# kamerkaya/SUPerman

Measured on AMD Instinct MI355X. Metric: Gray-code subset-steps/sec (dense n=40, d=0.5) at 1/2/4/8 MI355X; rel-err vs CPU, higher is better.
Workload: dtype f64; 1 GPU; dense Ryser/Gray-code exact permanent (-p4/-p6 path), n=40 d=0.50 (double/40_0.50_0), 2^39 Gray steps per step; n=40, kernel_request=dense, preprocessing=0, jit=1, walk=segmented (pattern-specialised), parallelism=dp1: contiguous wave-chunk shards + one RCCL all-reduce

## Files before the change

superman_amd/csrc/codescan.cpp:

```cpp
#include <amd_comgr/amd_comgr.h>
#include <elf.h>

#include <algorithm>
#include <cstring>
#include <map>
#include <string>
#include <string_view>
#include <vector>

#include "engine.hpp"

namespace sup {

namespace {

struct Inst {
  uint64_t addr = 0, size = 0;
  std::string text;
  int64_t target = -1;
};

struct DisCtx {
  const char* bytes = nullptr;
  uint64_t base = 0, len = 0;
// ... 66 lines not shown

bool starts(const std::string& s, const char* p) { return s.compare(0, std::strlen(p), p) == 0; }

bool is_f64_valu(const std::string& t) {
  return starts(t, "v_add_f64") || starts(t, "v_mul_f64") || starts(t, "v_fma_f64") || starts(t, "v_fmac_f64");
}
bool is_scratch(const std::string& t) { return starts(t, "scratch_") || starts(t, "buffer_"); }
bool is_readlane(const std::string& t) { return starts(t, "v_readlane"); }

}

int scan_code_object(const std::vector<char>& co, const char* kernel, CodeScan* out) {
  CodeScan r;
  r.vgprs = (int)meta_value(co, ".vgpr_count");
  r.vgpr_spills = (int)meta_value(co, ".vgpr_spill_count");
  r.scratch_bytes = (int)meta_value(co, ".private_segment_fixed_size");
  if (r.vgprs < 0 || r.vgpr_spills < 0 || r.scratch_bytes < 0) {
    set_error("code object: no register / scratch counts in its metadata");
    return SUP_EHIP;
  }
  const char* bytes = nullptr;
  uint64_t fa = 0, fs = 0, sa = 0, sl = 0;
  if (!find_function(co, kernel, &bytes, &fa, &fs, &sa, &sl) || fs == 0) {
    set_error(std::string("code object: kernel symbol ") + kernel + " not found");
    return SUP_EHIP;
  }
  DisCtx ctx;
  ctx.bytes = bytes, ctx.base = sa, ctx.len = sl;
  amd_comgr_disassembly_info_t dis;
  if (amd_comgr_create_disassembly_info("amdgcn-amd-amdhsa--gfx950", read_cb, print_cb, annot_cb, &dis) !=
      AMD_COMGR_STATUS_SUCCESS) {
    set_error("amd_comgr_create_disassembly_info failed");
    return SUP_EHIP;
  }
  std::vector<Inst> ins;
  int rc = SUP_OK;
  for (uint64_t a = fa; a < fa + fs;) {
    ctx.text.clear();
    ctx.target = -1;
    uint64_t sz = 0;
    if (amd_comgr_disassemble_instruction(dis, a, &ctx, &sz) != AMD_COMGR_STATUS_SUCCESS || sz == 0) {
      set_error("code object: disassembly failed");
      rc = SUP_EHIP;
      break;
    }
    Inst in;
    in.addr = a, in.size = sz;
    size_t p = ctx.text.find_first_not_of(" \t");
    in.text = p == std::string::npos ? std::string() : ctx.text.substr(p);
    const bool branch = starts(in.text, "s_branch") || starts(in.text, "s_cbranch");
    in.target = branch ? ctx.target : -1;
    ins.push_back(std::move(in));
    a += sz;
  }
  amd_comgr_destroy_disassembly_info(dis);
  if (rc) return rc;
  for (const Inst& in : ins) r.scratch_insts += is_scratch(in.text);
  r.insts = (int)ins.size();

  std::map<uint64_t, int> at;
  for (size_t i = 0; i < ins.size(); ++i) at[ins[i].addr] = (int)i;
  std::vector<char> leader(ins.size() + 1, 0);
  leader[0] = 1;
  for (size_t i = 0; i < ins.size(); ++i) {
    const Inst& in = ins[i];
    const bool ends = in.target >= 0 || starts(in.text, "s_endpgm") || starts(in.text, "s_setpc");
    if (ends) leader[i + 1] = 1;
    if (in.target >= 0) {
      auto it = at.find((uint64_t)in.target);
      if (it == at.end()) {
        set_error("code object: branch target outside the kernel");
        return SUP_EHIP;
      }
      leader[it->second] = 1;
    }
  }
  std::vector<int> bstart, block_of(ins.size());
  for (size_t i = 0; i < ins.size(); ++i) {
    if (leader[i]) bstart.push_back((int)i);
    block_of[i] = (int)bstart.size() - 1;
  }
  const int B = (int)bstart.size();
  std::vector<std::vector<int>> succ(B), pred(B);
  std::vector<int> bf64(B, 0), bscr(B, 0), blen(B, 0), brl(B, 0);
  for (int b = 0; b < B; ++b) {
    const int lo = bstart[b], hi = b + 1 < B ? bstart[b + 1] : (int)ins.size();
    for (int i = lo; i < hi; ++i)
      bf64[b] += is_f64_valu(ins[i].text), bscr[b] += is_scratch(ins[i].text), brl[b] += is_readlane(ins[i].text);
    blen[b] = hi - lo;
    const Inst& last = ins[hi - 1];
    auto add = [&](int to) {
      if (to >= 0 && to < B) succ[b].push_back(to), pred[to].push_back(b);
    };
    if (last.target >= 0) add(block_of[at[(uint64_t)last.target]]);
    const bool uncond = starts(last.text, "s_branch") || starts(last.text, "s_endpgm") || starts(last.text, "s_setpc");
    if (!uncond && hi < (int)ins.size()) add(b + 1);
  }
  std::vector<int> order, rpo_num(B, -1);
  {
    std::vector<char> seen(B, 0);
    std::vector<std::pair<int, size_t>> st{{0, 0}};
    seen[0] = 1;
    while (!st.empty()) {
      auto& [v, k] = st.back();
      if (k < succ[v].size()) {
        const int w = succ[v][k++];
        if (!seen[w]) seen[w] = 1, st.push_back({w, 0});
      } else {
        order.push_back(v);
        st.pop_back();
      }
    }
    std::reverse(order.begin(), order.end());
    for (size_t i = 0; i < order.size(); ++i) rpo_num[order[i]] = (int)i;
  }
  std::vector<int> idom(B, -1);
  idom[0] = 0;
  auto intersect = [&](int a, int b) {
    while (a != b) {
      while (rpo_num[a] > rpo_num[b]) a = idom[a];
      while (rpo_num[b] > rpo_num[a]) b = idom[b];
    }
    return a;
  };
  for (bool changed = true; changed;) {
    changed = false;
    for (int v : order) {
      if (v == 0) continue;
      int nd = -1;
      for (int p : pred[v])
        if (rpo_num[p] >= 0 && idom[p] >= 0) nd = nd < 0 ? p : intersect(p, nd);
      if (nd >= 0 && idom[v] != nd) idom[v] = nd, changed = true;
    }
  }
  auto dominates = [&](int h, int v) {
    if (rpo_num[v] < 0) return false;
    for (;;) {
      if (v == h) return true;
      if (v == 0) return false;
      v = idom[v];
    }
  };
  std::map<int, std::vector<char>> loops;
  for (int u = 0; u < B; ++u)
    for (int h : succ[u]) {
      if (!dominates(h, u)) continue;
      std::vector<char>& body = loops[h];
      if (body.empty()) body.assign(B, 0);
      body[h] = 1;
      std::vector<int> work;
      if (!body[u]) body[u] = 1, work.push_back(u);
      while (!work.empty()) {
        const int v = work.back();
        work.pop_back();
        for (int p : pred[v])
          if (!body[p]) body[p] = 1, work.push_back(p);
      }
    }
  r.loops = (int)loops.size();
  std::map<int, int> f64;
  for (auto& [h, body] : loops) {
    int s = 0;
    for (int b = 0; b < B; ++b) s += body[b] ? bf64[b] : 0;
    f64[h] = s;
  }
  int walk = -1;
  for (auto& [h, body] : loops) {
    bool outer = false;
    for (auto& [h2, body2] : loops)
      if (h2 != h && body[h2] && 2 * f64[h2] >= f64[h]) outer = true;
    if (!outer && (walk < 0 || f64[h] > f64[walk])) walk = h;
  }
  if (walk >= 0) {
    const std::vector<char>& body = loops[walk];
    r.loop_f64 = f64[walk];
    r.loop_scratch = 0;
    r.loop_insts = 0;
    r.loop_readlane = 0;
    for (int b = 0; b < B; ++b)
      if (body[b]) r.loop_scratch += bscr[b], r.loop_insts += blen[b], r.loop_readlane += brl[b];
  }
  *out = r;
  return SUP_OK;
}

}
```

superman_amd/csrc/engine.hpp:

```cpp
#pragma once
#include <stdint.h>
#include <cstdio>
#include <memory>
#include <mutex>
#include <functional>
#include <string>
#include <vector>

#include "../../include/superman.h"
#include "kernels.hpp"

namespace sup {

void set_error(const std::string& msg);
const char* last_error();
bool env_on(const char* name, bool dflt);

int to_double(const void* mat, sup_dtype t, int n, std::vector<double>& out);

void nw_start(const double* A, int n, double* x0, double* p0);

constexpr int kMaxCachedBits = 4;

enum SegCensus {
  kCenXAdd = 0,
  kCenCopy,
  kCenOuter,
  kCenInner,
  kCenD,
  kCenAcc,
  kCenLane,
  kCenSharedAdd,
  kCenSharedCopy,
  kCenSharedForm,
  kCenHiAdd,
  kCenHiCopy,
  kCenHiForm,
  kCenStart,
  kSegCensusN
};

struct Layout {
  int L;
  int m;
  int h;
  bool fixed = false;
  int cc_cap = kMaxCachedBits;
  uint64_t chunks() const { return 1ull << h; }
};
Layout default_layout(int n);
Layout layout_with_walk(int n, int walk_log2);

struct ProdTree {
  std::vector<int> item_row;
  std::vector<uint32_t> item_sig;
  int tail_lo = 0, tail_hi = 0;
  std::vector<int> a, b;
  std::vector<uint32_t> sig;
  std::vector<uint8_t> item_live, node_live;
  int items() const { return (int)item_row.size(); }
  int K() const { return (int)a.size(); }
  int root() const { return K() ? items() + K() - 1 : (items() ? 0 : -1); }
  uint32_t root_sig() const { return K() ? sig.back() : (items() ? item_sig[0] : 0u); }
};

struct Plan {
  int n = 0;
  int NP = 0;
  WalkKind kind = kWalkDense;
  Layout lay{};
  std::vector<int> rowperm;
  std::vector<int> colmap;
  std::vector<double> cols;
  std::vector<double> x0;
  std::vector<int> nblk;
  std::vector<uint64_t> rowmask;
  uint64_t umask = 0;
  uint64_t chunk_ends = 0;
  std::vector<int> seg_start;
  std::vector<std::vector<int>> touched;
  std::vector<int> sub_start;
  int seg_b = 0;
  std::vector<int> dyn_rows;
  ProdTree outer_tree;
  ProdTree inner_tree;
  bool lds = false;
  bool integral = false;
  int seg_cc = 0;
  double seg_ops = 0.0;
  double seg_model_ops = 0.0;
  int seg_hi = 0;
  double seg_census[kSegCensusN] = {};
  double seg_skip = 0.0;
  int seg_regs = 0;
  int seg_budget = 0;
  std::vector<int> jofs;
  std::vector<double> jtab;
  size_t seg_cbase = 0;
  bool start_tab_on = false;
  std::vector<double> start_tab;
  int seg_kp = 4;
  std::string jit_src;
  uint64_t jit_key = 0;
  uint64_t uid = 0;
  std::vector<int> seg_order;
  bool seg_loop_scratch = false;
};

struct SegChoice {
  std::vector<int> order;
  int b = 0;
  int budget = 0;
  int cc_cap = kMaxCachedBits;
  int hi = 0;
};

int make_plan(const double* A, int n, WalkKind kind, bool identity_map, const Layout& lay, Plan& P,
              const SegChoice* choice = nullptr);

std::vector<int> greedy_walk_order(const double* A, int n, int count);
bool skip_walk_order(const double* A, int n, const Layout& lay, std::vector<int>& out,
                     const std::vector<int>* baseline, double factor);
int improve_sparse_plan(const double* A, int n, const Layout& lay, Plan& P);
int plan_threads();

std::vector<int> seg_walk_order(const double* A, int n, int m, int count, int* b_out, int cc_cap = kMaxCachedBits);
double seg_skip_estimate(const double* A, int n, const std::vector<int>& order, int m, int samples);
double seg_skip_fraction_plan(const Plan& P, int samples);
std::vector<int> seg_row_order(const double* A, int n, const std::vector<int>& walk);
int build_seg(Plan& P, int fixed_budget = 0, int fixed_hi = 0);
bool seg_choice_load(uint64_t key, int* m, SegChoice* c);
bool seg_choice_exists(uint64_t key);
double seg_cold_model(int n);
double seg_cold_predict(int n);
void seg_cost_store(int n, double seconds);
double seg_cost_ratio_load();
void seg_choice_store(uint64_t key, int m, const SegChoice& c);
int auto_decision_load(uint64_t key);
int auto_decision_store(uint64_t key, int seg);
uint64_t jit_toolchain_hash();
int seg_static_bits(int m);
double seg_cx(const Plan& P, int r, uint32_t S);
double seg_cy(const Plan& P, int r, uint32_t S);
double seg_walk_cost(const Plan& P);
int jit_occupancy(int dev, const Plan& P, int* blocks_per_cu, double* compile_ms);
int jit_launch(int dev, const Plan& P, const WalkParams& p, int grid, hipStream_t s);
int jit_compile_only(const Plan& P, double* compile_ms);
struct CodeScan {
  int vgprs = -1, vgpr_spills = -1, scratch_bytes = -1;
  int insts = 0, scratch_insts = 0, loops = 0;
  int loop_scratch = -1, loop_f64 = 0, loop_insts = 0;
  int loop_readlane = 0;
};
int scan_code_object(const std::vector<char>& code, const char* kernel, CodeScan* out);
int jit_code_scan(const Plan& P, CodeScan* out);
double jit_compile_ms_thread();

double walk_cost(const Plan& P);
double walk_seconds(const Plan& P, double steps);

int plan_for(const double* A, int n, sup_kernel kernel, const Layout& lay, Plan& P, int jit = -1, int ndev = 1,
             int dev = 0);
int plan_for_shared(const double* A, int n, sup_kernel kernel, const Layout& lay, std::shared_ptr<const Plan>& P,
                    int jit = -1, int ndev = 1, int dev = 0, bool keep = true);

struct RangeResult {
  double partial = 0.0;
  double kernel_ms = 0.0;
  uint64_t visited = 0;
  int grid = 0;
  double compile_ms = 0.0;
};

int run_item_queue(uint64_t nitems, int takers, const std::function<int(int, uint64_t)>& take);
int run_range(int dev, const Plan& P, uint64_t c0, uint64_t c1, bool want_visited, RangeResult& r,
              double* slot = nullptr);
struct LaunchGeom {
  unsigned group, tail_group;
  uint64_t tail_begin, grid;
  unsigned tail_ticket;
};
LaunchGeom walk_geometry(uint64_t count, uint64_t resident_blocks, uint64_t waves_per_block, bool seg,
                         int force_group = 0, int force_tail = -1, uint64_t group_cap = 64);
constexpr int kMaxBatchLeaves = 32;
constexpr int kMaxBatchLeafChunkBits = 26;
static_assert((uint64_t)kMaxBatchLeaves << kMaxBatchLeafChunkBits <= (1ull << 32),
              "leaf batches must fit 32-bit chunk indices");
bool batchable(const Plan& a, const Plan& b);
int run_range_batch(int dev, const std::vector<const Plan*>& plans, std::vector<double>& partial, double* kernel_ms);

double pairwise_host(const std::vector<double>& v);

int device_count(int* n);
constexpr int kCtxLanes = 8;
void set_ctx_lane(int lane);
int ctx_lane();
void set_defer_timing(bool on);
int kernel_time(int dev, double* total_ms, uint64_t* launches);
int phys_device(int dev);
hipError_t select_device(int dev);
int check_device(int dev, const char* what);
uint64_t device_checks_passed();
#ifndef SUP_HIP
#define SUP_HIP(call)                                                                  \
  do {                                                                                 \
    hipError_t e_ = (call);                                                            \
    if (e_ != hipSuccess) {                                                            \
      set_error(std::string(#call) + ": " + hipGetErrorString(e_));                    \
      return SUP_EHIP;                                                                 \
    }                                                                                  \
  } while (0)
#endif

#define SUP_ON_DEVICE(dev, what)                 \
  do {                                           \
    const int rc_ = check_device((dev), (what)); \
    if (rc_) return rc_;                         \
  } while (0)
int warm_devices(int first, int count, int n);
int rccl_physical_devices(const std::vector<int>& devs, std::vector<int>& phys);

struct SchedResult {
  double total = 0.0;
  double kernel_ms = 0.0;
  uint64_t visited = 0;
  int devices = 0;
  int grid = 0;
  int cpu_items = 0;
  double compile_ms = 0.0;
  int items_resumed = 0;
  std::vector<double> dev_partials;
};
int schedule(const Plan& P, sup_sched sched, const sup_opts& o, uint64_t c0, uint64_t c1,
             SchedResult& out);
struct Checkpoint {
// ... 223 lines not shown
```

superman_amd/csrc/jit.cpp:

```cpp
#include <dlfcn.h>
#include <hip/hiprtc.h>
#include <sched.h>
#include <spawn.h>
#include <sys/stat.h>
#include <sys/wait.h>
#include <unistd.h>

#include <cerrno>

#include <algorithm>
#include <cstring>
#include <fstream>
#include <iterator>
#include <atomic>
#include <chrono>
#include <cmath>
#include <cstdio>
#include <cstdlib>
#include <map>
#include <queue>
#include <memory>
#include <condition_variable>
#include <mutex>
#include <sstream>
// ... 228 lines not shown
    const double bd = best < 0 ? 0.0 : dlt[best];
    if (!took_hi && (best < 0 || (bd > 1e-9 && regs <= budget_hi))) out(*fit_hi, ops, regs), took_hi = true;
    if (best < 0 || (bd > 1e-9 && regs <= budget)) break;
    heap.pop();
    V[best].live = false;
    ++ver[best];
    ops += bd, regs -= V[best].store;
    for (int p = V[best].parent; p >= 0; p = V[p].parent) {
      V[p].F += (double)V[p].cop / V[best].cop * V[best].F;
      if (V[p].live) {
        push(p);
        break;
      }
    }
    stack.assign(1, best);
    while (!stack.empty()) {
      const int u = stack.back();
      stack.pop_back();
      for (int k : V[u].kids)
        if (k >= 0) {
          if (V[k].live) push(k);
          else stack.push_back(k);
        }
    }
  }
  if (!took_hi) out(*fit_hi, ops, regs);
  out(f, ops, regs);
  return f;
}

std::atomic<long> g_fit_calls{0};
int search_budget() {
  static const int b = std::getenv("SUP_JIT_SEARCH_BUDGET") ? std::atoi(std::getenv("SUP_JIT_SEARCH_BUDGET")) : kRegsMax;
  return b;
}

int max_cached() {
  const char* e = std::getenv("SUP_JIT_MAXCC");
  return e ? std::max(0, std::min(kMaxCachedBits, std::atoi(e))) : kMaxCachedBits;
}

SegFit seg_best(const SegRows& R, int cc_max, int regs_max = kRegsMax) {
  ++g_fit_calls;
  SegFit best;
  double bscore = 1e300;
  for (int cc = 0; cc <= std::min(cc_max, std::max(0, R.b - 1)); ++cc) {
    SegFit hi;
    SegFit lo = seg_fit(R, cc, kRegs3, regs_max, &hi);
    for (SegFit* f : {&lo, &hi}) {
      if (f->regs > regs_max && cc > 0) continue;
      const double score = f->ops * (f->regs <= kRegs3 ? 1.0 : kOcc2Penalty) * (f->regs > regs_max ? 2.0 : 1.0);
      if (score < bscore) bscore = score, best = std::move(*f);
    }
  }
  return best;
}

SegRows seg_rows_of(const double* A, int n, const std::vector<int>& walk, int b) {
  SegRows R;
  R.n = n, R.m = (int)walk.size();
  const std::vector<int> order = seg_row_order(A, n, walk);
  auto nz = [&](int row, int c) { return A[(size_t)row * n + c] != 0.0; };
  R.touched.assign(R.m, {});
  std::vector<char> any1(n, 0);
  for (int k = 0; k < R.m; ++k)
    for (int j = 0; j < n; ++j)
      if (nz(order[j], walk[k])) {
        R.touched[k].push_back(j);
        if (k >= 1) any1[j] = 1;
      }
  R.len0 = (int)R.touched[0].size();
  R.s_end = 0;
  while (R.s_end < R.len0 && any1[R.s_end]) ++R.s_end;
  R.r_end = R.len0;
  while (R.r_end < n && any1[R.r_end]) ++R.r_end;
  seg_rows_finish(R, b);
  return R;
}

double seg_score(const SegFit& f) { return f.ops * (f.regs <= kRegs3 ? 1.0 : kOcc2Penalty); }

constexpr double kMaxBlockBytes = 40.0 * 1024.0;
double seg_block_bytes(const SegFit& f, int b) { return 1.25 * 8.0 * 2.0 * f.ops * (double)(1u << b); }

std::vector<int> seg_b_candidates(int m) {
  std::vector<int> v;
  if (const char* e = std::getenv("SUP_JIT_B")) {
    v.push_back(std::min(m - 1, std::max(3, std::min(8, std::atoi(e)))));
    return v;
  }
  for (int b = 5; b <= 8; ++b) {
    const int bb = std::min(m - 1, b);
    if (v.empty() || v.back() != bb) v.push_back(bb);
  }
  return v;
}

}

int seg_static_bits(int m) {
  int b = 5;
  if (const char* e = std::getenv("SUP_JIT_B")) b = std::max(3, std::min(8, std::atoi(e)));
  return std::min(m - 1, b);
}

double seg_walk_cost(const Plan& P) { return P.seg_ops; }

int plan_threads() {
  int t = (int)std::max(1u, std::thread::hardware_concurrency());
  if (const char* e = std::getenv("OMP_NUM_THREADS")) t = std::min(t, std::max(1, std::atoi(e)));
  return std::min(t, 16);
}

void parallel_tasks(size_t count, const std::function<void(size_t)>& fn, int max_threads = 1 << 20) {
  std::atomic<size_t> next{0};
  auto worker = [&]() {
    for (size_t i = next++; i < count; i = next++) fn(i);
  };
  std::vector<std::thread> th;
  for (int t = 1; t < std::min({plan_threads(), (int)count, max_threads}); ++t) th.emplace_back(worker);
  worker();
  for (auto& t : th) t.join();
}

int seg_search_starts(int n) {
  if (const char* e = std::getenv("SUP_JIT_STARTS")) return std::max(1, std::atoi(e));
  return std::ldexp(1.0, n - 1) * (2.0 * n + 1.0) / 3.7e13 >= 1.0 ? 32 : 3;
}

std::vector<int> seg_walk_order(const double* A, int n, int m, int count, int* b_out, int cc_cap) {
  cc_cap = std::min(cc_cap, max_cached());
  const int nb = n - 1;
  m = std::min(m, nb);
  count = std::min(std::max(count, m), nb);
  std::vector<int> nnz(n, 0);
  for (int c = 0; c < nb; ++c)
    for (int i = 0; i < n; ++i) nnz[c] += A[(size_t)i * n + c] != 0.0;
  auto extend = [&](std::vector<int> order, int upto) {
    std::vector<char> used(n, 0), placed(n, 0);
    for (int c : order) {
      used[c] = 1;
      for (int i = 0; i < n; ++i) placed[i] |= A[(size_t)i * n + c] != 0.0;
    }
    while ((int)order.size() < upto) {
      int best = -1, bnew = 1 << 30;
      for (int c = 0; c < nb; ++c) {
        if (used[c]) continue;
        int nw = 0;
        for (int i = 0; i < n; ++i) nw += !placed[i] && A[(size_t)i * n + c] != 0.0;
        if (nw < bnew || (nw == bnew && nnz[c] < nnz[best])) best = c, bnew = nw;
      }
      used[best] = 1;
      order.push_back(best);
      for (int i = 0; i < n; ++i) placed[i] |= A[(size_t)i * n + best] != 0.0;
    }
    return order;
  };
  auto cost = [&](const std::vector<int>& o, int b) {
    if (nnz[o[0]] == 0) return 1e300;
    if (m < 3) return 0.0;
    const SegFit f = seg_best(seg_rows_of(A, n, std::vector<int>(o.begin(), o.begin() + m), b), cc_cap,
                              search_budget());
    return seg_block_bytes(f, b) > kMaxBlockBytes ? 1e300 : seg_score(f);
  };
  if (m == 0) {
    if (b_out) *b_out = 0;
// ... 936 lines not shown
    auto tree_init = [&](int ti, int v) {
      const ProdTree& t = tr(ti);
      if (t.tail_hi > t.tail_lo)
        o << "      const double " << (ti == 0 ? "Ro" : (v ? "Cy" : "Cx")) << " = "
          << tree(t.tail_lo, t.tail_hi, v ? "y" : "x") << ";\n";
      for (int i = 0; i < t.K(); ++i)
        if (this->nlive(ti, v, i))
          for (uint32_t S : submasks(t.sig[i] & ccm))
            o << "      double " << nname(ti, v, i, S) << " = " << iopnd(ti, v, t.a[i], S) << " * "
              << iopnd(ti, v, t.b[i], S) << ";\n";
    };
    tree_init(0, 0);
    o << "      double acc = 0.0;\n";
    o << "      uint32_t vis = 0;\n";
    if (P.outer_tree.tail_hi > P.outer_tree.tail_lo)
      o << "      if (__builtin_amdgcn_ballot_w64(SUP_LANE() < " << (1u << L) << "u && Ro != 0.0) != 0) {\n";
    else
      o << "      {\n";
    o << "      vis = " << (1u << m) << "u;\n";
    tree_init(1, 0);
    tree_init(1, 1);
    if (P.inner_tree.root() >= 0)
      for (uint32_t S : submasks(inner_root_csig()))
        o << "      double " << dname(S) << " = " << dexpr([&](int v, int id) { return iopnd(1, v, id, S); })
          << ";\n";
    else
      o << "      double D0 = 0.0;\n";
    {
      const std::string U = top(0, 0, 0);
      o << "      acc = " << (U.empty() ? dname(0) : dname(0) + " * " + U) << ";\n";
    }
    o << "      double tot = 0.0;\n";
    if (trace) o << "      asm volatile(\"\" : \"+v\"(acc));\n      tr_sc += __builtin_amdgcn_s_memtime() - tr_s;\n      ++tr_n;\n";
    const int u = std::max(0, std::min(P.seg_hi, m - 1 - b));
    const unsigned U = 1u << u;
    const size_t start_end = o.str().size();
    if (u > 0) {
      hi_loop(Q, U, u);
    } else {
    o << "      for (uint32_t q = 0; q < " << Q << "u; ++q) {\n";
    const char* ind = "        ";
    o << ind << "const char* jt = (const char*)opaque_c(p.jtab, 0u);\n";
    o << ind << "const uint32_t ng = q & 1u;\n";
    {
      std::vector<Item> items;
      for (unsigned st = 1; st < B; ++st) {
        const int pb = __builtin_ctz(st), k = pb + 1;
        if (pb >= cc && !P.touched[k].empty())
          step_items(items, "jt", pb < b - 1 ? off_const(k, (st >> (pb + 1)) & 1u) : off_dyn(k, "ng"),
                     P.touched[k], false, step_class(k, b));
        items.push_back({accumulate_text(st & 1u, state(st)), {}});
        body[kCenAcc] += 1.0;
      }
      emit_items(items, ind);
    }
    body[kCenAcc] += 1.0;
    if (Q > 1) {
      o << ind << "if (q + 1u < " << Q << "u) {\n";
      o << ind << "  const uint32_t kk = (uint32_t)__builtin_ctz(q + 1u);\n";
      o << ind << "  const uint32_t ngd = ((q + 1u) >> (kk + 1u)) & 1u;\n";
      {
        std::vector<Item> items;
        step_items(items, "(const char*)opaque_c(p.cols, 0u)",
                   "(2u * (" + std::to_string(L + b + 1) + "u + kk) + ngd) * " + std::to_string(P.NP * 8) + "u",
                   P.dyn_rows, true, P.seg_b, kSharedStep);
        items.push_back({accumulate_text(false, 0u), {}});
        emit_items(items, "          ");
      }
      o << ind << "  tot += acc;\n" << ind << "  acc = 0.0;\n";
      body[kCenLane] += 1.0;
      o << ind << "}\n";
    }
    o << "      }\n";
    }
    {
      const double steps = 2.0 * (double)U * (double)B;
      double walk = 0.0;
      for (int c = 0; c < kCenStart; ++c) census[c] = body[c] / steps, walk += body[c];
      const std::string init = o.str().substr(start_begin, start_end - start_begin);
      const double start_ops = count_sub(init, " + ") + count_sub(init, " * ") + count_sub(init, " - ") +
                               count_sub(init, "__builtin_fma(") + 7.0 +
                               (double)n * ((double)L + (P.start_tab_on ? 0.0 : 0.5 * (double)(n - 1 - L - m)));
      census[kCenStart] = std::ldexp(start_ops, -m);
      block_bytes = 1.25 * 8.0 * walk;
    }
    o << "      acc = tot + acc;\n";
    o << "      if (((uint32_t)ga ^ (uint32_t)__builtin_popcount(SUP_LANE())) & 1u) acc = -acc;\n";
    o << "      }\n";
    o << "      const uint32_t lane = SUP_LANE();\n";
    o << "      const double part = wave_sum(lane < " << (1u << L) << "u ? acc : 0.0);\n";
    o << "      if (lane == j) s_keep[wv][j] = part, s_vkeep[wv][j] = vis;\n";
    o << "    }\n";
    o << "    __builtin_amdgcn_fence(__ATOMIC_RELEASE, \"wavefront\");\n";
    o << "    __builtin_amdgcn_wave_barrier();\n";
    o << "    __builtin_amdgcn_fence(__ATOMIC_ACQUIRE, \"wavefront\");\n";
    o << "    const uint32_t lane = SUP_LANE();\n";
    o << "    chunk_store(base, len, s_keep[wv][lane], s_vkeep[wv][lane]);\n";
    o << "    __builtin_amdgcn_wave_barrier();\n";
    o << "  }\n";
    if (trace)
      o << "  if (p.trace && SUP_LANE() == 0) {\n"
        << "    unsigned long long* t = p.trace + 8ull * (blockIdx.x * " << kBlock / 64 << "u + wv);\n"
        << "    t[0] = tr_r0; t[1] = __builtin_amdgcn_s_memrealtime(); t[2] = tr_c0;\n"
        << "    t[3] = __builtin_amdgcn_s_memtime(); t[4] = tr_n; t[5] = tr_sc;\n"
        << "  }\n";
    o << "}\n";
    o << "}  // namespace sup\n";
    return o.str();
  }
};

const char* const kJitOpts[] = {"--offload-arch=gfx950", "-O3", "-std=c++17", "-ffp-contract=off"};
constexpr int kJitNopts = 4;

}

std::vector<std::string> jit_opts() {
  std::vector<std::string> v(kJitOpts, kJitOpts + kJitNopts);
  if (const char* e = std::getenv("SUP_JIT_SCHED"))
    if (*e) v.push_back("-mllvm"), v.push_back(std::string("-amdgpu-sched-strategy=") + e);
  if (const char* e = std::getenv("SUP_JIT_OPAQUE_R2"))
    if (std::atoi(e)) v.push_back("-DSUP_OPAQUE_BEFORE_OFFSET=1");
  return v;
}

namespace {

uint64_t fnv1a(const std::string& s, uint64_t h = 1469598103934665603ull) {
  for (unsigned char c : s) h = (h ^ c) * 1099511628211ull;
  return h;
}

std::string hiprtc_version() {
  static const std::string v = [] {
    int major = 0, minor = 0;
    if (hiprtcVersion(&major, &minor) != HIPRTC_SUCCESS) return std::string("hiprtc ?");
    std::string r = "hiprtc " + std::to_string(major) + "." + std::to_string(minor) + " hip " + std::to_string(HIP_VERSION);
    Dl_info di;
    if (dladdr(reinterpret_cast<void*>(&hiprtcCreateProgram), &di) && di.dli_fname) {
      const char* slash = std::strrchr(di.dli_fname, '/');
      r += std::string(" ") + (slash ? slash + 1 : di.dli_fname);
      std::ifstream f(di.dli_fname, std::ios::binary);
      if (f) {
        std::string bytes((std::istreambuf_iterator<char>(f)), std::istreambuf_iterator<char>());
        char hx[40];
        std::snprintf(hx, sizeof hx, " %zu %016llx", bytes.size(), (unsigned long long)fnv1a(bytes));
        r += hx;
      }
    }
    return r;
  }();
  return v;
}

}

uint64_t toolchain_hash_impl() {
  std::string key;
  for (const std::string& opt : jit_opts()) key += "\n//" + opt;
  key += std::string("\n//") + kWalkCommonSrc + kWalkParamsSrc;
  key += "\n//" + hiprtc_version();
  return fnv1a(key);
}

namespace {

uint64_t jit_source_key(const std::string& src) {
// ... 24 lines not shown
        for (int j = 0; j < n; ++j) x[j] += col[j];
      }
    }
  });
}

int build_seg(Plan& P, int fixed_budget, int fixed_hi) {
  const int n = P.n, L = P.lay.L, m = P.lay.m;
  if (m < 3) {
    set_error("segmented walk needs >= 3 walk bits");
    return SUP_EINVAL;
  }
  if (P.cols.empty()) return SUP_EINVAL;
  P.start_tab.clear();
  P.start_tab_on = !std::getenv("SUP_JIT_NO_START_TAB") && P.lay.m <= kStartTabMaxWalkBits &&
                   (double)P.lay.chunks() * P.NP * sizeof(double) <= (double)kStartTabMaxBytes;
  P.touched.assign(m, {});
  P.seg_start.assign(1, 0);
  std::vector<char> seen(n, 0);
  int R = 0;
  for (int k = 0; k < m; ++k) {
    const double* col = P.cols.data() + (size_t)(2 * (L + k)) * P.NP;
    for (int j = 0; j < n; ++j)
      if (col[j] != 0.0) {
        P.touched[k].push_back(j);
        if (!seen[j]) seen[j] = 1, ++R;
      }
    if (R > P.seg_start.back()) P.seg_start.push_back(R);
  }
  for (int j = 0; j < R; ++j)
    if (!seen[j]) {
      set_error("segmented walk: rows are not in first-touch order");
      return SUP_EINVAL;
    }
  if (P.touched[0].empty()) {
    set_error("segmented walk: walk column 0 has no nonzero");
    return SUP_EINVAL;
  }
  {
    const int len0 = P.seg_start[1];
    std::vector<char> got(len0, 0);
    int cnt = 0;
    P.sub_start.assign(1, 0);
    for (int k = 1; k < m; ++k) {
      for (int r : P.touched[k])
        if (r < len0 && !got[r]) {
          if (r != cnt) {
            set_error("segmented walk: segment 0 rows are not in sub-segment order");
            return SUP_EINVAL;
          }
          got[r] = 1, ++cnt;
        }
      if (cnt > P.sub_start.back()) P.sub_start.push_back(cnt);
    }
  }
  if (P.seg_b < 1 || P.seg_b > m - 1) {
    P.seg_b = seg_static_bits(m);
    if (!std::getenv("SUP_JIT_B")) {
      double best = 1e300;
      for (const int cb : seg_b_candidates(m)) {
        SegRows R;
        R.n = n, R.m = m, R.touched = P.touched;
        R.len0 = P.seg_start[1], R.s_end = P.sub_start.back(), R.r_end = P.seg_start.back();
        seg_rows_finish(R, cb);
        const SegFit f = seg_best(R, std::min(max_cached(), P.lay.cc_cap));
        const double sc = seg_block_bytes(f, cb) > kMaxBlockBytes ? 1e300 : seg_score(f);
        if (sc < best - 1e-12) best = sc, P.seg_b = cb;
      }
    }
  }
  P.dyn_rows.clear();
  {
    std::vector<char> in(n, 0);
    for (int k = P.seg_b + 1; k < m; ++k)
      for (int r : P.touched[k]) in[r] = 1;
    for (int j = 0; j < n; ++j)
      if (in[j]) P.dyn_rows.push_back(j);
  }
  SegRows SR;
  SR.n = n, SR.m = m, SR.touched = P.touched;
  SR.len0 = P.seg_start[1], SR.s_end = P.sub_start.back(), SR.r_end = P.seg_start.back();
  seg_rows_finish(SR, P.seg_b);
  const int cc_cap = std::min(max_cached(), P.lay.cc_cap);
  auto finish = [&SR, &cc_cap, n, L, m](Plan& Q, int budget, int hi) {
    SegFit f;
    if (const char* e = std::getenv("SUP_JIT_CC"))
      f = seg_fit(SR, std::max(0, std::min({std::atoi(e), SR.b - 1, kMaxCachedBits})), budget);
    else f = seg_best(SR, cc_cap, budget);
    if (const char* e = std::getenv("SUP_JIT_STORAGE")) f = seg_fit(SR, f.cc, std::max(0, std::atoi(e)));
    Q.outer_tree = std::move(f.outer);
    Q.inner_tree = std::move(f.inner);
    Q.seg_cc = f.cc;
    Q.seg_model_ops = f.ops;
    Q.seg_regs = f.regs;
    Q.seg_budget = budget;
    Q.jofs.assign(m, 0);
    Q.jtab.clear();
    for (int k = 0; k < m; ++k) {
      const std::vector<int>& t = Q.touched[k];
      const size_t blk = (t.size() + 7) & ~(size_t)7;
      Q.jofs[k] = (int)Q.jtab.size();
      Q.jtab.resize(Q.jtab.size() + 2 * std::max<size_t>(blk, 8), 0.0);
      for (size_t i = 0; i < t.size(); ++i) {
        Q.jtab[Q.jofs[k] + i] = Q.cols[(size_t)(2 * (L + k)) * Q.NP + t[i]];
        Q.jtab[Q.jofs[k] + blk + i] = Q.cols[(size_t)(2 * (L + k) + 1) * Q.NP + t[i]];
      }
    }
    Q.seg_cbase = Q.jtab.size();
    Q.seg_kp = 4;
    if (const char* e = std::getenv("SUP_JIT_KP")) Q.seg_kp = std::max(1, std::atoi(e));
    const int hi_max = std::min(3, m - 1 - Q.seg_b);
    if (const char* e = std::getenv("SUP_JIT_HI")) hi = std::max(0, std::min(3, std::atoi(e)));
    bool neg_zero = false;
    for (int j = 0; j < n; ++j) neg_zero = neg_zero || (Q.x0[j] == 0.0 && std::signbit(Q.x0[j]));
    if (neg_zero) hi = 0;
    auto generate = [&Q](int h, std::string* src) {
      Q.seg_hi = h;
      auto g = std::make_unique<Gen>(Q);
      *src = g->source();
      return g;
    };
    auto total = [](const Gen& g) {
      double ops = 0.0;
      for (int c = 0; c < kCenStart; ++c) ops += g.census[c];
      return ops;
    };
    int taken = hi < 0 ? 0 : std::min(hi, hi_max);
    std::string src;
    std::unique_ptr<Gen> g = generate(taken, &src);
    for (int h = hi < 0 ? hi_max : 0; h > 0; --h) {
      std::string s2;
      std::unique_ptr<Gen> gh = generate(h, &s2);
      if (gh->block_bytes <= kMaxBlockBytes && total(*gh) < total(*g)) {
        g = std::move(gh), src = std::move(s2), taken = h;
        break;
      }
    }
    Q.seg_hi = taken;
    Q.jit_src = std::move(src);
    for (int c = 0; c < kSegCensusN; ++c) Q.seg_census[c] = g->census[c];
    Q.seg_ops = total(*g);
    {
      const std::vector<double> t = g->tail();
      Q.jtab.insert(Q.jtab.end(), t.begin(), t.end());
    }
    Q.jit_key = jit_source_key(Q.jit_src);
  };
  const char* env_budget = std::getenv("SUP_JIT_BUDGET");
  const int hi_unchecked = fixed_budget > 0 ? fixed_hi : 0;
  if (env_budget) fixed_budget = std::max(1, std::atoi(env_budget));
  finish(P, fixed_budget > 0 ? fixed_budget : kRegsMax, hi_unchecked);
  const bool fixed = fixed_budget > 0 || std::getenv("SUP_JIT_REGMAX") || std::getenv("SUP_JIT_STORAGE") ||
                     std::getenv("SUP_JIT_CC") || std::getenv("SUP_JIT_NOVERIFY");
  const double walk_s = std::ldexp(1.0, n - 1) * P.seg_ops / 3.7e13;
  if (fixed && std::getenv("SUP_JIT_VERBOSE")) {
    CodeScan s;
    const int rc = jit_code_scan(P, &s);
    std::fprintf(stderr, "  fixed budget %d: ops %.4f rc %d vgprs %d spills %d scratch %dB (loop %d of %d insts)\n",
                 P.seg_budget, P.seg_ops, rc, s.vgprs, s.vgpr_spills, s.scratch_bytes, s.loop_scratch, s.loop_insts);
  }
  if (!fixed && walk_s < 0.01 && P.seg_cc > 3) {
    CodeScan s;
    P.seg_loop_scratch = jit_code_scan(P, &s) != SUP_OK || s.loop_scratch != 0;
  }
  auto ladder = [&](int hi, Plan& out) -> int {
    std::vector<int> budgets;
    for (int b2 = kRegs3 + 12; b2 <= kRegsMax + 60; b2 += 8) budgets.push_back(b2);
    std::vector<Plan> cand(budgets.size(), P);
    parallel_tasks(budgets.size(), [&](size_t i) { finish(cand[i], budgets[i], hi); });
    std::vector<size_t> idx;
    for (size_t i = 0; i < cand.size(); ++i) {
      bool dup = false;
      for (size_t j : idx) dup = dup || cand[j].jit_key == cand[i].jit_key;
      if (!dup) idx.push_back(i);
    }
    std::vector<CodeScan> scans(cand.size());
    std::vector<int> src(cand.size(), SUP_EHIP);
    std::vector<char> done(cand.size(), 0);
    auto compile_one = [&](size_t i) {
      if (done[i]) return;
      const auto t0 = std::chrono::steady_clock::now();
      const double own = t_compile_ms;
      src[i] = jit_code_scan(cand[i], &scans[i]);
      t_compile_ms = own + std::chrono::duration<double, std::milli>(std::chrono::steady_clock::now() - t0).count();
      done[i] = 1;
    };
    auto clean = [&](size_t i) { return done[i] && src[i] == SUP_OK && scans[i].loop_scratch == 0; };
    size_t pp = 0;
    for (size_t k = 0; k < idx.size(); ++k)
      if (budgets[idx[k]] <= kRegsMax) pp = k;
    enum { kUnknown = 0, kFail, kDirty, kCleanScratch, kClean0 };
    constexpr long kLadderDone = -1, kLadderFail = -2;
    auto next_needed = [&](const std::vector<int>& o) -> long {
      const size_t probe = idx[pp];
      if (o[probe] == kUnknown) return (long)probe;
      if (o[probe] == kFail) return kLadderFail;
      auto cl = [&](size_t i) { return o[i] >= kCleanScratch; };
      size_t c_pos;
      if (cl(probe)) {
        size_t lo = pp, hi = idx.size();
        while (hi - lo > 1) {
          const size_t mid = lo + (hi - lo) / 2;
          if (o[idx[mid]] == kUnknown) return (long)idx[mid];
          (cl(idx[mid]) ? lo : hi) = mid;
        }
        c_pos = lo;
      } else {
        long lo = -1, hi = (long)pp;
        while (hi - lo > 1) {
          const long mid = lo + (hi - lo) / 2;
          if (o[idx[mid]] == kUnknown) return (long)idx[mid];
          (cl(idx[mid]) ? lo : hi) = mid;
        }
        if (lo < 0) return kLadderFail;
        c_pos = (size_t)lo;
      }
      if (o[idx[c_pos]] != kClean0)
        for (size_t k = c_pos; k-- > 0;) {
          if (cand[idx[k]].seg_ops > cand[idx[c_pos]].seg_ops * (1.0 + kScratchTolerance)) break;
          if (o[idx[k]] == kUnknown) return (long)idx[k];
          if (o[idx[k]] == kClean0) break;
        }
      return kLadderDone;
    };
    std::vector<int> outcome(cand.size(), kUnknown);
    const size_t procs = rtc_procs();
    for (;;) {
      const long k = next_needed(outcome);
      if (k < 0) break;
      if (procs > 1 && !jit_code_cached(cand[k])) {
        std::vector<const Plan*> batch;
        std::vector<char> queued(cand.size(), 0);
        std::queue<std::vector<int>> q;
        q.push(outcome);
        for (size_t visits = 0; !q.empty() && batch.size() < procs && visits < 4096; ++visits) {
          std::vector<int> h = std::move(q.front());
          q.pop();
          const long s = next_needed(h);
          if (s < 0) continue;
          if (!queued[s] && !jit_code_cached(cand[s])) queued[s] = 1, batch.push_back(&cand[s]);
          for (int r : {kDirty, kCleanScratch, kClean0}) {
            std::vector<int> h2 = h;
            h2[s] = r;
            q.push(std::move(h2));
          }
        }
        const auto t0 = std::chrono::steady_clock::now();
        prefetch_compiles(batch, procs);
        t_compile_ms += std::chrono::duration<double, std::milli>(std::chrono::steady_clock::now() - t0).count();
      }
      compile_one((size_t)k);
      outcome[k] = src[k] != SUP_OK         ? kFail
                   : scans[k].loop_scratch  ? kDirty
                   : scans[k].scratch_bytes ? kCleanScratch
                                            : kClean0;
    }
    if (outcome[idx[pp]] == kFail) return (int)SUP_EHIP;
    auto pick = [&]() {
      int c = -1, bare = -1;
      for (size_t i : idx) {
        if (!clean(i)) continue;
        if (c < 0 || cand[i].seg_ops < cand[c].seg_ops) c = (int)i;
        if (scans[i].scratch_bytes == 0 && (bare < 0 || cand[i].seg_ops < cand[bare].seg_ops)) bare = (int)i;
      }
      return (bare >= 0 && c >= 0 && cand[bare].seg_ops <= cand[c].seg_ops * (1.0 + kScratchTolerance)) ? bare : c;
    };
    const int best = pick();
    if (std::getenv("SUP_JIT_VERBOSE"))
      for (size_t i : idx)
        if (done[i])
          std::fprintf(stderr, "  budget %d hi %d: ops %.4f rc %d vgprs %d spills %d scratch %dB (loop %d of %d insts, %d readlane)%s\n",
                       budgets[i], cand[i].seg_hi, cand[i].seg_ops, src[i], scans[i].vgprs, scans[i].vgpr_spills,
                       scans[i].scratch_bytes, scans[i].loop_scratch, scans[i].loop_insts, scans[i].loop_readlane,
                       (int)i == best ? "  <- chosen" : "");
    if (best < 0) {
      set_error("segmented walk: every budget's kernel touches scratch inside its walk loop (or fails to compile)");
      return (int)SUP_EHIP;
    }
    out = std::move(cand[best]);
    return SUP_OK;
  };
  if (!fixed && walk_s >= 0.01 && P.seg_regs > kRegs3) {
    Plan best_hi, best_0;
    const int rc_hi = ladder(-1, best_hi);
    int rc_0 = SUP_EHIP;
    bool need_0 = rc_hi != SUP_OK || best_hi.seg_hi == 0;
    if (!need_0) {
      Plan top = P;
      finish(top, kRegsMax + 60, 0);
      need_0 = top.seg_ops <= best_hi.seg_ops;
    }
    if (rc_hi == SUP_OK && best_hi.seg_hi == 0) rc_0 = SUP_OK, best_0 = best_hi, need_0 = false;
    else if (need_0) rc_0 = ladder(0, best_0);
    if (rc_hi != SUP_OK && rc_0 != SUP_OK) return SUP_EHIP;
    const bool take_hi = rc_hi == SUP_OK && (rc_0 != SUP_OK || best_hi.seg_ops < best_0.seg_ops);
    if (std::getenv("SUP_JIT_VERBOSE"))
      std::fprintf(stderr, "  high-bit steps: %s (unrolled ladder %s hi %d ops %.4f; plain ladder %s ops %.4f)\n",
                   take_hi ? "taken" : "not taken", rc_hi == SUP_OK ? "ok" : "failed", best_hi.seg_hi,
                   rc_hi == SUP_OK ? best_hi.seg_ops : 0.0,
                   rc_0 == SUP_OK ? "ok" : (need_0 ? "failed" : "not needed"), rc_0 == SUP_OK ? best_0.seg_ops : 0.0);
    P = std::move(take_hi ? best_hi : best_0);
  }
  P.seg_skip = seg_skip_fraction_plan(P, 2048);
  if (P.start_tab_on) seg_start_table(P);
  if (std::getenv("SUP_JIT_VERBOSE"))
    std::fprintf(stderr, "seg plan n=%d m=%d b=%d ops/step=%.4f regs=%d cc=%d table=%zu B (columns %zu B) key=%016llx "
                 "(storage plans evaluated: %ld)\n", n, m, P.seg_b, P.seg_ops, P.seg_regs, P.seg_cc,
                 P.jtab.size() * sizeof(double), P.seg_cbase * sizeof(double), (unsigned long long)P.jit_key,
                 g_fit_calls.load());
  if (std::getenv("SUP_JIT_VERBOSE")) {
    const double* c = P.seg_census;
    std::fprintf(stderr,
                 "  op census (fp64 ops per Gray step, hi=%d): x adds %.4f, copy adds %.4f, outer forms %.4f, "
                 "segment-0 forms %.4f, D %.4f, accumulates %.4f, lane sum %.4f, shared step adds %.4f copies %.4f "
                 "forms %.4f, high-bit steps adds %.4f copies %.4f forms %.4f; total %.4f (storage fit's count of the "
                 "plain walk loop without the lane sum %.4f); beside it, chunk start %.4f\n",
                 P.seg_hi, c[kCenXAdd], c[kCenCopy], c[kCenOuter], c[kCenInner], c[kCenD], c[kCenAcc], c[kCenLane],
                 c[kCenSharedAdd], c[kCenSharedCopy], c[kCenSharedForm], c[kCenHiAdd], c[kCenHiCopy], c[kCenHiForm],
                 P.seg_ops, P.seg_model_ops, c[kCenStart]);
  }
  return SUP_OK;
}

std::string seg_source(const Plan& P, int kp) {
  Plan Q = P;
  Q.seg_kp = kp;
  return Gen(Q).source();
}

}
```

superman_amd/csrc/plan.cpp:

```cpp
#include "engine.hpp"

#include <algorithm>
#include <atomic>
#include <chrono>
#include <cmath>
#include <cstdio>
#include <cstdlib>
#include <cstring>
#include <map>
#include <memory>
#include <mutex>
#include <thread>
#include <tuple>

#include <unistd.h>

namespace sup {

static thread_local std::string g_err;
void set_error(const std::string& msg) { g_err = msg; }
const char* last_error() { return g_err.c_str(); }

bool env_on(const char* name, bool dflt) {
  const char* e = std::getenv(name);
// ... 392 lines not shown
      for (int i = 0; i < n; ++i)
        if (!placed[i] && A[(size_t)i * n + c] != 0.0) {
          placed[i] = 1;
          order.push_back(i);
        }
      P.nblk[L + k] = ((int)order.size() + 7) / 8;
    }
    for (int i = 0; i < n; ++i)
      if (!placed[i]) order.push_back(i);
    P.rowperm = order;
    if (kind == kWalkSeg) {
      std::vector<int> walk(m);
      for (int k = 0; k < m; ++k) walk[k] = P.colmap[L + k];
      P.rowperm = seg_row_order(A, n, walk);
    }
  }
  for (int e = 0; e < nb; ++e)
    if (e < L || e >= L + m) P.nblk[e] = (n + 7) / 8;

  P.cols.assign((size_t)2 * std::max(nb, 1) * P.NP, 0.0);
  for (int e = 0; e < nb; ++e) {
    const int c = P.colmap[e];
    for (int j = 0; j < n; ++j) {
      const double v = A[(size_t)P.rowperm[j] * n + c];
      P.cols[(size_t)(2 * e) * P.NP + j] = v;
      P.cols[(size_t)(2 * e + 1) * P.NP + j] = -v;
    }
  }
  std::vector<double> x0(n);
  double p0;
  nw_start(A, n, x0.data(), &p0);
  P.x0.assign(P.NP, 0.0);
  for (int j = 0; j < n; ++j) P.x0[j] = x0[P.rowperm[j]];

  P.umask = 0;
  for (int j = 0; j < n; ++j) {
    const int i = P.rowperm[j];
    bool lane_touched = false;
    for (int e = 0; e < L; ++e)
      if (A[(size_t)i * n + P.colmap[e]] != 0.0) lane_touched = true;
    if (!lane_touched) P.umask |= 1ull << j;
    uint64_t rm = 0;
    for (int k = 0; k < m; ++k)
      if (A[(size_t)i * n + P.colmap[L + k]] != 0.0) rm |= 1ull << k;
    P.rowmask[j] = rm;
    if ((kind == kWalkSparse || kind == kWalkDense) && !lane_touched && rm == 0 && !no_chunk_ends())
      P.chunk_ends |= 1ull << j;
  }
  if (kind == kWalkSeg) return build_seg(P, choice ? choice->budget : 0, choice ? choice->hi : 0);
  return SUP_OK;
}

static constexpr double kJitMinSavingSec = 3.0;
static constexpr double kAutoRuns = 4.0;
static constexpr double kJitWarmSavingSec = 0.1;
static constexpr int kJitWarmMinN = 30;

static int plan_for_uncached(const double* A, int n, sup_kernel kernel, const Layout& lay, Plan& P, int jit,
                             int ndev, int dev, double min_saving);
static double auto_min_saving(const double* A, int n, const Layout& lay, int jit);

static constexpr double kSegStartOps = 2048.0;

static constexpr int kSegMinChunkBits = 14;

static uint64_t knob_hash() {
  Fnv1a f;
  for (char** e = environ; e && *e; ++e) {
    const char* v = *e;
    if (std::strncmp(v, "SUP_JIT_", 8) != 0 || !std::strncmp(v, "SUP_JIT_CACHE_DIR=", 18) ||
        !std::strncmp(v, "SUP_JIT_DUMP=", 13) || !std::strncmp(v, "SUP_JIT_VERBOSE=", 16) ||
        !std::strncmp(v, "SUP_JIT_COLD_RATIO=", 19))
      continue;
    f.bytes(v, std::strlen(v));
    f.bytes("\xff", 1);
  }
  return f.h;
}

static uint64_t seg_disk_key(const double* A, int n, const Layout& lay) {
  Fnv1a f{0x5eed5e9a11ull ^ jit_toolchain_hash()};
  const size_t nn = (size_t)n * n;
  const bool integral = is_integral(A, n);
  const int32_t head[] = {7 , n, lay.L, lay.m, (int32_t)lay.fixed, (int32_t)integral};
  f.bytes(head, sizeof head);
  if (integral) {
    f.bytes(A, nn * sizeof(double));
  } else {
    std::vector<unsigned char> pat((nn + 7) / 8, 0);
    for (size_t i = 0; i < nn; ++i)
      if (A[i] != 0.0) pat[i / 8] |= (unsigned char)(1u << (i % 8));
    f.bytes(pat.data(), pat.size());
  }
  const uint64_t k = knob_hash();
  f.bytes(&k, sizeof k);
  return f.h;
}

static int make_seg_plan(const double* A, int n, const Layout& lay, Plan& P) {
  const uint64_t dkey = seg_disk_key(A, n, lay);
  {
    int m2 = 0;
    SegChoice c;
    if (seg_choice_load(dkey, &m2, &c) && m2 >= 3 && m2 <= lay.m + lay.h && (!lay.fixed || m2 == lay.m)) {
      Layout l2 = lay;
      l2.m = m2;
      l2.h = lay.m + lay.h - m2;
      l2.cc_cap = c.cc_cap;
      if (make_plan(A, n, kWalkSeg, false, l2, P, &c) == SUP_OK) return SUP_OK;
    }
  }
  const auto t_cold = std::chrono::steady_clock::now();
  auto plan = [A, n](const Layout& l, Plan& Q) {
    int r = make_plan(A, n, kWalkSeg, false, l, Q);
    if (r == SUP_OK && Q.seg_loop_scratch && l.cc_cap > 3) {
      Layout l3 = l;
      l3.cc_cap = 3;
      r = make_plan(A, n, kWalkSeg, false, l3, Q);
    }
    return r;
  };
  int rc = plan(lay, P);
  if (rc) return rc;
  if (!lay.fixed) {
    const int mmax = std::min(lay.m + lay.h - kSegMinChunkBits, 31);
    int m2 = lay.m;
    while (m2 < mmax && std::ldexp(P.seg_model_ops, m2) < 32.0 * kSegStartOps) ++m2;
    if (m2 != lay.m) {
      Layout l2 = lay;
      l2.m = m2;
      l2.h = lay.m + lay.h - m2;
      Plan s2;
      if (plan(l2, s2) == SUP_OK) {
        auto eff = [](const Plan& q) {
          return (1.0 - q.seg_skip) * (q.seg_model_ops + std::ldexp(kSegStartOps, -q.lay.m));
        };
        if (eff(s2) < eff(P)) P = std::move(s2);
      }
    }
  }
  SegChoice c;
  c.order = P.seg_order;
  c.b = P.seg_b;
  c.budget = P.seg_budget;
  c.hi = P.seg_hi;
  c.cc_cap = P.lay.cc_cap;
  seg_choice_store(dkey, P.lay.m, c);
  const double cold_s = std::chrono::duration<double>(std::chrono::steady_clock::now() - t_cold).count();
  seg_cost_store(n, cold_s);
  if (std::getenv("SUP_JIT_VERBOSE"))
    std::fprintf(stderr, "cold segmented plan n=%d: %.3f s (compiles %.3f s wall on this thread)\n", n, cold_s,
                 jit_compile_ms_thread() * 1e-3);
  return SUP_OK;
}

namespace {
struct PlanKey {
  uint64_t hash;
  int n, kernel, L, m, jit, ndev;
  bool fixed;
  uint64_t knobs;
  bool operator<(const PlanKey& o) const {
    return std::tie(hash, n, kernel, L, m, jit, ndev, fixed, knobs) <
           std::tie(o.hash, o.n, o.kernel, o.L, o.m, o.jit, o.ndev, o.fixed, o.knobs);
  }
};
std::mutex g_plan_mu;
// ... 225 lines not shown
```

Baseline: 3254 billion gray-steps/s.

## Search high-bit unroll depth with descending ladders and raise loop body byte cap

The planner's body-size estimate now uses a calibrated bytes-per-op constant with a larger 52 KiB cap, so deeper high-bit unrolls are allowed where they were previously rejected. The old two-ladder choice (unrolled vs plain) becomes a descending search over unroll caps u, each ladder filtered to plans no worse in ops than the current best, with ties broken by smaller body bytes. Code-scan also reports loop body bytes for diagnostics. Larger loop bodies can cut per-step fp64 ops, but they risk instruction-cache pressure and add plan-time compile work.

After: 3283 billion gray-steps/s (median of 6 runs). No clear change (+0.9%).

```diff
diff --git a/superman_amd/csrc/codescan.cpp b/superman_amd/csrc/codescan.cpp
--- a/superman_amd/csrc/codescan.cpp
+++ b/superman_amd/csrc/codescan.cpp
@@ -172,12 +172,13 @@
   }
   const int B = (int)bstart.size();
   std::vector<std::vector<int>> succ(B), pred(B);
-  std::vector<int> bf64(B, 0), bscr(B, 0), blen(B, 0), brl(B, 0);
+  std::vector<int> bf64(B, 0), bscr(B, 0), blen(B, 0), brl(B, 0), bbytes(B, 0);
   for (int b = 0; b < B; ++b) {
     const int lo = bstart[b], hi = b + 1 < B ? bstart[b + 1] : (int)ins.size();
     for (int i = lo; i < hi; ++i)
       bf64[b] += is_f64_valu(ins[i].text), bscr[b] += is_scratch(ins[i].text), brl[b] += is_readlane(ins[i].text);
     blen[b] = hi - lo;
+    bbytes[b] = (int)(ins[hi - 1].addr + ins[hi - 1].size - ins[lo].addr);
     const Inst& last = ins[hi - 1];
     auto add = [&](int to) {
       if (to >= 0 && to < B) succ[b].push_back(to), pred[to].push_back(b);
@@ -267,8 +268,10 @@
     r.loop_scratch = 0;
     r.loop_insts = 0;
     r.loop_readlane = 0;
+    r.loop_bytes = 0;
     for (int b = 0; b < B; ++b)
-      if (body[b]) r.loop_scratch += bscr[b], r.loop_insts += blen[b], r.loop_readlane += brl[b];
+      if (body[b])
+        r.loop_scratch += bscr[b], r.loop_insts += blen[b], r.loop_readlane += brl[b], r.loop_bytes += bbytes[b];
   }
   *out = r;
   return SUP_OK;
diff --git a/superman_amd/csrc/engine.hpp b/superman_amd/csrc/engine.hpp
--- a/superman_amd/csrc/engine.hpp
+++ b/superman_amd/csrc/engine.hpp
@@ -90,6 +90,7 @@
   double seg_ops = 0.0;
   double seg_model_ops = 0.0;
   int seg_hi = 0;
+  double seg_body_bytes = 0.0;
   double seg_census[kSegCensusN] = {};
   double seg_skip = 0.0;
   int seg_regs = 0;
@@ -151,6 +152,7 @@
   int insts = 0, scratch_insts = 0, loops = 0;
   int loop_scratch = -1, loop_f64 = 0, loop_insts = 0;
   int loop_readlane = 0;
+  int loop_bytes = 0;
 };
 int scan_code_object(const std::vector<char>& code, const char* kernel, CodeScan* out);
 int jit_code_scan(const Plan& P, CodeScan* out);
diff --git a/superman_amd/csrc/jit.cpp b/superman_amd/csrc/jit.cpp
--- a/superman_amd/csrc/jit.cpp
+++ b/superman_amd/csrc/jit.cpp
@@ -334,6 +334,9 @@
 
 constexpr double kMaxBlockBytes = 40.0 * 1024.0;
 double seg_block_bytes(const SegFit& f, int b) { return 1.25 * 8.0 * 2.0 * f.ops * (double)(1u << b); }
+
+constexpr double kBodyBytesPerOp = 8.5;
+constexpr double kMaxBodyBytes = 52.0 * 1024.0;
 
 std::vector<int> seg_b_candidates(int m) {
   std::vector<int> v;
@@ -1436,7 +1439,7 @@
                                count_sub(init, "__builtin_fma(") + 7.0 +
                                (double)n * ((double)L + (P.start_tab_on ? 0.0 : 0.5 * (double)(n - 1 - L - m)));
       census[kCenStart] = std::ldexp(start_ops, -m);
-      block_bytes = 1.25 * 8.0 * walk;
+      block_bytes = kBodyBytesPerOp * walk;
     }
     o << "      acc = tot + acc;\n";
     o << "      if (((uint32_t)ga ^ (uint32_t)__builtin_popcount(SUP_LANE())) & 1u) acc = -acc;\n";
@@ -1627,7 +1630,7 @@
   SR.len0 = P.seg_start[1], SR.s_end = P.sub_start.back(), SR.r_end = P.seg_start.back();
   seg_rows_finish(SR, P.seg_b);
   const int cc_cap = std::min(max_cached(), P.lay.cc_cap);
-  auto finish = [&SR, &cc_cap, n, L, m](Plan& Q, int budget, int hi) {
+  auto finish = [&SR, &cc_cap, n, L, m](Plan& Q, int budget, int hi, int cap = 3) {
     SegFit f;
     if (const char* e = std::getenv("SUP_JIT_CC"))
       f = seg_fit(SR, std::max(0, std::min({std::atoi(e), SR.b - 1, kMaxCachedBits})), budget);
@@ -1655,7 +1658,7 @@
     Q.seg_kp = 4;
     if (const char* e = std::getenv("SUP_JIT_KP")) Q.seg_kp = std::max(1, std::atoi(e));
     const int hi_max = std::min(3, m - 1 - Q.seg_b);
-    if (const char* e = std::getenv("SUP_JIT_HI")) hi = std::max(0, std::min(3, std::atoi(e)));
+    if (const char* e = std::getenv("SUP_JIT_HI")) hi = std::max(-1, std::min(3, std::atoi(e)));
     bool neg_zero = false;
     for (int j = 0; j < n; ++j) neg_zero = neg_zero || (Q.x0[j] == 0.0 && std::signbit(Q.x0[j]));
     if (neg_zero) hi = 0;
@@ -1673,10 +1676,10 @@
     int taken = hi < 0 ? 0 : std::min(hi, hi_max);
     std::string src;
     std::unique_ptr<Gen> g = generate(taken, &src);
-    for (int h = hi < 0 ? hi_max : 0; h > 0; --h) {
+    for (int h = hi < 0 ? std::min(hi_max, cap) : 0; h > 0; --h) {
       std::string s2;
       std::unique_ptr<Gen> gh = generate(h, &s2);
-      if (gh->block_bytes <= kMaxBlockBytes && total(*gh) < total(*g)) {
+      if (gh->block_bytes <= kMaxBodyBytes && total(*gh) < total(*g)) {
         g = std::move(gh), src = std::move(s2), taken = h;
         break;
       }
@@ -1685,6 +1688,7 @@
     Q.jit_src = std::move(src);
     for (int c = 0; c < kSegCensusN; ++c) Q.seg_census[c] = g->census[c];
     Q.seg_ops = total(*g);
+    Q.seg_body_bytes = g->block_bytes;
     {
       const std::vector<double> t = g->tail();
       Q.jtab.insert(Q.jtab.end(), t.begin(), t.end());
@@ -1701,24 +1705,29 @@
   if (fixed && std::getenv("SUP_JIT_VERBOSE")) {
     CodeScan s;
     const int rc = jit_code_scan(P, &s);
-    std::fprintf(stderr, "  fixed budget %d: ops %.4f rc %d vgprs %d spills %d scratch %dB (loop %d of %d insts)\n",
-                 P.seg_budget, P.seg_ops, rc, s.vgprs, s.vgpr_spills, s.scratch_bytes, s.loop_scratch, s.loop_insts);
+    std::fprintf(stderr, "  fixed budget %d hi %d: ops %.4f rc %d vgprs %d spills %d scratch %dB (loop %d of %d insts, %d B; "
+                 "counted %.0f B)\n", P.seg_budget, P.seg_hi, P.seg_ops, rc, s.vgprs, s.vgpr_spills, s.scratch_bytes,
+                 s.loop_scratch, s.loop_insts, s.loop_bytes, P.seg_body_bytes);
   }
   if (!fixed && walk_s < 0.01 && P.seg_cc > 3) {
     CodeScan s;
     P.seg_loop_scratch = jit_code_scan(P, &s) != SUP_OK || s.loop_scratch != 0;
   }
-  auto ladder = [&](int hi, Plan& out) -> int {
+  auto ladder = [&](int cap, double ops_max, Plan& out, int* u_seen) -> int {
     std::vector<int> budgets;
     for (int b2 = kRegs3 + 12; b2 <= kRegsMax + 60; b2 += 8) budgets.push_back(b2);
     std::vector<Plan> cand(budgets.size(), P);
-    parallel_tasks(budgets.size(), [&](size_t i) { finish(cand[i], budgets[i], hi); });
+    parallel_tasks(budgets.size(), [&](size_t i) { finish(cand[i], budgets[i], -1, cap); });
     std::vector<size_t> idx;
+    *u_seen = 0;
     for (size_t i = 0; i < cand.size(); ++i) {
+      *u_seen = std::max(*u_seen, cand[i].seg_hi);
+      if (cand[i].seg_ops > ops_max) continue;
       bool dup = false;
       for (size_t j : idx) dup = dup || cand[j].jit_key == cand[i].jit_key;
       if (!dup) idx.push_back(i);
     }
+    if (idx.empty()) return (int)SUP_EHIP;
     std::vector<CodeScan> scans(cand.size());
     std::vector<int> src(cand.size(), SUP_EHIP);
     std::vector<char> done(cand.size(), 0);
@@ -1814,10 +1823,11 @@
     if (std::getenv("SUP_JIT_VERBOSE"))
       for (size_t i : idx)
         if (done[i])
-          std::fprintf(stderr, "  budget %d hi %d: ops %.4f rc %d vgprs %d spills %d scratch %dB (loop %d of %d insts, %d readlane)%s\n",
+          std::fprintf(stderr, "  budget %d hi %d: ops %.4f rc %d vgprs %d spills %d scratch %dB (loop %d of %d insts, %d B; "
+                       "counted %.0f B, %d readlane)%s\n",
                        budgets[i], cand[i].seg_hi, cand[i].seg_ops, src[i], scans[i].vgprs, scans[i].vgpr_spills,
-                       scans[i].scratch_bytes, scans[i].loop_scratch, scans[i].loop_insts, scans[i].loop_readlane,
-                       (int)i == best ? "  <- chosen" : "");
+                       scans[i].scratch_bytes, scans[i].loop_scratch, scans[i].loop_insts, scans[i].loop_bytes,
+                       cand[i].seg_body_bytes, scans[i].loop_readlane, (int)i == best ? "  <- chosen" : "");
     if (best < 0) {
       set_error("segmented walk: every budget's kernel touches scratch inside its walk loop (or fails to compile)");
       return (int)SUP_EHIP;
@@ -1826,25 +1836,39 @@
     return SUP_OK;
   };
   if (!fixed && walk_s >= 0.01 && P.seg_regs > kRegs3) {
-    Plan best_hi, best_0;
-    const int rc_hi = ladder(-1, best_hi);
-    int rc_0 = SUP_EHIP;
-    bool need_0 = rc_hi != SUP_OK || best_hi.seg_hi == 0;
-    if (!need_0) {
-      Plan top = P;
-      finish(top, kRegsMax + 60, 0);
-      need_0 = top.seg_ops <= best_hi.seg_ops;
-    }
-    if (rc_hi == SUP_OK && best_hi.seg_hi == 0) rc_0 = SUP_OK, best_0 = best_hi, need_0 = false;
-    else if (need_0) rc_0 = ladder(0, best_0);
-    if (rc_hi != SUP_OK && rc_0 != SUP_OK) return SUP_EHIP;
-    const bool take_hi = rc_hi == SUP_OK && (rc_0 != SUP_OK || best_hi.seg_ops < best_0.seg_ops);
-    if (std::getenv("SUP_JIT_VERBOSE"))
-      std::fprintf(stderr, "  high-bit steps: %s (unrolled ladder %s hi %d ops %.4f; plain ladder %s ops %.4f)\n",
-                   take_hi ? "taken" : "not taken", rc_hi == SUP_OK ? "ok" : "failed", best_hi.seg_hi,
-                   rc_hi == SUP_OK ? best_hi.seg_ops : 0.0,
-                   rc_0 == SUP_OK ? "ok" : (need_0 ? "failed" : "not needed"), rc_0 == SUP_OK ? best_0.seg_ops : 0.0);
-    P = std::move(take_hi ? best_hi : best_0);
+    Plan best;
+    int u_seen = 0;
+    int rc_best = ladder(3, 1e300, best, &u_seen);
+    std::string trail;
+    if (std::getenv("SUP_JIT_VERBOSE")) {
+      char t[96];
+      std::snprintf(t, sizeof t, "u <= %d %s", u_seen, rc_best == SUP_OK ? "" : "failed");
+      trail = t;
+      if (rc_best == SUP_OK) std::snprintf(t, sizeof t, "u %d budget %d ops %.4f", best.seg_hi, best.seg_budget, best.seg_ops), trail += t;
+    }
+    for (int u2 = (rc_best == SUP_OK ? best.seg_hi : u_seen) - 1; u2 >= 0 && !std::getenv("SUP_JIT_HI"); --u2) {
+      if (rc_best == SUP_OK) {
+        Plan top = P;
+        finish(top, kRegsMax + 60, -1, u2);
+        if (top.seg_ops > best.seg_ops) break;
+      }
+      Plan c;
+      int seen2 = 0;
+      const int rc = ladder(u2, rc_best == SUP_OK ? best.seg_ops : 1e300, c, &seen2);
+      const bool take = rc == SUP_OK && (rc_best != SUP_OK || c.seg_ops < best.seg_ops ||
+                                         (c.seg_ops == best.seg_ops && c.seg_body_bytes < best.seg_body_bytes));
+      if (std::getenv("SUP_JIT_VERBOSE")) {
+        char t[128];
+        if (rc == SUP_OK) std::snprintf(t, sizeof t, "; u <= %d: u %d budget %d ops %.4f%s", u2, c.seg_hi, c.seg_budget, c.seg_ops, take ? " (taken)" : "");
+        else std::snprintf(t, sizeof t, "; u <= %d: none", u2);
+        trail += t;
+      }
+      if (take) best = std::move(c), rc_best = SUP_OK;
+      u2 = std::min(u2, seen2);
+    }
+    if (rc_best != SUP_OK) return SUP_EHIP;
+    if (std::getenv("SUP_JIT_VERBOSE")) std::fprintf(stderr, "  high-bit steps: ladders %s -> u %d\n", trail.c_str(), best.seg_hi);
+    P = std::move(best);
   }
   P.seg_skip = seg_skip_fraction_plan(P, 2048);
   if (P.start_tab_on) seg_start_table(P);
diff --git a/superman_amd/csrc/plan.cpp b/superman_amd/csrc/plan.cpp
--- a/superman_amd/csrc/plan.cpp
+++ b/superman_amd/csrc/plan.cpp
@@ -498,7 +498,7 @@
   Fnv1a f{0x5eed5e9a11ull ^ jit_toolchain_hash()};
   const size_t nn = (size_t)n * n;
   const bool integral = is_integral(A, n);
-  const int32_t head[] = {7 , n, lay.L, lay.m, (int32_t)lay.fixed, (int32_t)integral};
+  const int32_t head[] = {8 , n, lay.L, lay.m, (int32_t)lay.fixed, (int32_t)integral};
   f.bytes(head, sizeof head);
   if (integral) {
     f.bytes(A, nn * sizeof(double));
```
